# andrewmilson/ecfft

Hardware: AMD Instinct MI355X
Metric: secp256k1 Fp field-mul/s, ENTER+EXIT at n=2^20 (higher is better)
Workload: dtype u256; 1 GPU; secp256k1::Fp n=2^20 ENTER+EXIT (BASELINE.json configs[2]); n=1048576, field=secp256k1, parallelism=1 independent polynomial(s), one per GPU, no collective, inputs=device-resident (HBM) before the timed region, steps=449, warmup=5

## Files before the change

### ecfft_amd/csrc/device_tree.h

```cpp
#pragma once
#include <hip/hip_runtime.h>
#include <vector>
#include <set>
#include <map>
#include <mutex>
#include <atomic>
#include <cstdio>
#include <cstdlib>
#include <new>
#include <algorithm>
#include "kernels.h"
#include "host_curve.h"
#include "transport.h"

namespace ecfft {

#ifdef ECFFT_TEST_HOOKS
inline const char* ab_env(const char* name) { return getenv(name); }
#else
inline const char* ab_env(const char*) { return nullptr; }
#endif

#define ECFFT_HIP_TRY(x)                                                                   \
    do { hipError_t e_ = (x); if (e_ != hipSuccess) {                                      \
// ... 51 lines not shown

#define ECFFT_LAUNCH(cls, alg_bytes, kern, grid, block, lds, stream, ...)               \
    do { if (prof_.on) prof_.begin(stream, cls, (double)(alg_bytes));                  \
         hipLaunchKernelGGL(kern, grid, block, lds, stream, __VA_ARGS__);               \
         if (prof_.on) prof_.end(stream); } while (0)

#ifndef ECFFT_BATCH_SPLIT
#define ECFFT_BATCH_SPLIT 1
#endif
#ifndef ECFFT_SYM_BFLY
#define ECFFT_SYM_BFLY 1
#endif
#ifndef ECFFT_BATCH_WAYS
#define ECFFT_BATCH_WAYS 2
#endif
template <class F>
class DeviceChain {
public:
    using E = typename F::elem;
    using TE = typename F::telem;
    using Tree = LevelTables<F>;

    ~DeviceChain() { release(); }

    size_t size() const { return N_; }
    unsigned log_size() const { return L_; }
    const Tree& tree(unsigned log_m) const { return trees_[log_m]; }
    const Tree& tree_at(unsigned log_m) const { return (ovr_tree_ && ovr_tree_->log_m == log_m) ? *ovr_tree_ : trees_[log_m]; }
    const HostTree<F>& host() const { return host_; }
    int exit_cores() const { return exit3_ ? 3 : 4; }
    int exit_low_cores() const { return exit3_ && kExitLowForm == 3 && !exit_low4_ ? 3 : 4; }
    int sym_bfly() const { return !sym_ ? 0 : (sym_general_kernels_ ? 2 : 1); }
    int low_sym() const { return (kLowSymEnter && low_sym_enter() ? 1 : 0) | (kLowSymExit && low_sym_exit() ? 2 : 0); }
    int low_map(int dir) const {
        if (trees_.size() > 5 && trees_[5].low32_A[dir]) return 32;
        if (trees_.size() > 4 && trees_[4].low16_A[dir]) return 16;
        return 0;
    }
    const E* f_device() const { return f_; }
    std::mutex& lock() { return mu_; }
#ifdef ECFFT_TEST_HOOKS
    static std::atomic<int>& test_fail_build_rank() { static std::atomic<int> r{-1}; return r; }
#endif
    Profiler& profiler() const { return prof_; }

    bool build(HostTree<F>&& ht, int device) {
        host_ = std::move(ht);
        N_ = host_.n; L_ = ilog2(N_); device_ = device;
        ECFFT_HIP_TRY(hipSetDevice(device_));
        hipStream_t s = nullptr;
        size_t total = 2 * N_ + 64 + 2 * (L_ ? L_ : 1) + 64;
        for (unsigned l = 0; l <= L_; ++l) total += (6 + 11 * kTeElems) * ((size_t)1 << l) + 1024 + blk16_elems(l);
        if (!exit4_) for (unsigned l = 1; l <= L_; ++l) total += (l <= kLogLow ? 6 : 1) * kTeElems * ((size_t)1 << l) / 2 + 64;
        total += low16_elems();
        ECFFT_HIP_TRY(hipMalloc(&arena_, total * sizeof(E)));
        arena_cap_ = total; arena_used_ = 0;
        f_ = take(2 * N_);
        if (!points_on_device(f_, s)) { fprintf(stderr, "ecfft: point set construction failed\n"); return false; }
        if (!exit4_) {
            unsigned long long* zc = nullptr; unsigned long long hz = 0;
            ECFFT_HIP_TRY(hipMalloc(&zc, sizeof(unsigned long long)));
            (void)hipMemsetAsync(zc, 0, sizeof(unsigned long long), s);
            const E* leaves = f_ + N_;
            foreach_n(s, N_, [=] __device__(size_t j) { if (F::is_zero(leaves[j])) atomicAdd(zc, 1ull); });
            const bool got = hipMemcpyAsync(&hz, zc, sizeof(hz), hipMemcpyDeviceToHost, s) == hipSuccess && hipStreamSynchronize(s) == hipSuccess;
            (void)hipFree(zc);
// ... 471 lines not shown
            batch_inv(xqe, xqei, hc, s); batch_inv(xqo, xqoi, hc, s);
            foreach_n(s, hc, [=] __device__(size_t j) {
                e0[j] = F::mul(F::sub(F::sqr(xe[j]), zc0[j]), xqei[j]);
                e1[j] = F::mul(F::sub(F::sqr(F::sub(zb[j], xo[j])), zc1[j]), xqoi[j]);
            });
            ok = modred_split(tr, base, lq, m, e0, e1, h0, h1, xqei, xqo, 1, zib, 1, zc0, zc1, 1, t0, x0, x1, A, B, s, true);
            if (!ok) break;
            foreach_n(s, hc, [=] __device__(size_t j) { c0[j] = F::mul_add(xqe[j], h0[j], zc0[j]); c1[j] = F::mul_add(xqo[j], h1[j], zc1[j]); });
            E* z1s = temp(hc);
            pointwise_z(lm, 1, (size_t)a, hc, z1s, fdev, lc_inv, s, Q);
            foreach_n(s, hc, [=] __device__(size_t j) { e0[j] = F::sqr(F::sub(z1s[j], xe[j])); e1[j] = F::sqr(xo[j]); });
            ok = modred_split(tr, base, lq, m, e0, e1, q0, q1, xei, xo, 1, zib, 1, c0, c1, 1, t0, x0, x1, A, B, s, true);
            if (!ok) break;
            pz0[0] = c0; pz0[1] = c1; pz1[0] = q0; pz1[1] = q1;
            if (hipStreamSynchronize(s) != hipSuccess) { ok = false; break; }
            temps_free();
        }
        ok = ok && hipGetLastError() == hipSuccess && hipStreamSynchronize(s) == hipSuccess;
        temps_free();
        ok = tr.vote(ok, s);
        if (!ok) { fprintf(stderr, "ecfft: sharded EXIT table build failed\n"); return false; }
        host_.f.clear(); host_.f.shrink_to_fit();
        ECFFT_HIP_TRY(hipMalloc(&d_trees_, (L_ + 1) * sizeof(Tree)));
        ECFFT_HIP_TRY(hipMemcpy(d_trees_, trees_.data(), (L_ + 1) * sizeof(Tree), hipMemcpyHostToDevice));
        return true;
    }

#ifndef ECFFT_LOG_TILE_BYTES
#define ECFFT_LOG_TILE_BYTES 15
#endif
#ifndef ECFFT_CT_ALL
#define ECFFT_CT_ALL 0
#endif
    static constexpr unsigned kLogTileMax = (sizeof(E) == 32) ? ECFFT_LOG_TILE_BYTES - 5 : ECFFT_LOG_TILE_BYTES - 2;
#ifndef ECFFT_COL_STAGES
#define ECFFT_COL_STAGES 9
#endif
#ifndef ECFFT_LOG_COL_TILE_BYTES
#define ECFFT_LOG_COL_TILE_BYTES 15
#endif
#ifndef ECFFT_COL_MIN_LOGC
#define ECFFT_COL_MIN_LOGC 1
#endif
#ifndef ECFFT_COL_STAGES_4B
#define ECFFT_COL_STAGES_4B 9
#endif
    static constexpr unsigned kColStages = sizeof(E) == 4 ? ECFFT_COL_STAGES_4B : ECFFT_COL_STAGES;
    static constexpr bool kSymKernels = sizeof(E) == 32 && ECFFT_SYM_BFLY != 0;
    static constexpr bool kLowSymEnter = kSymKernels && ECFFT_ENTER_LOW_SYM != 0;
    static constexpr unsigned kLogColTileMax = (sizeof(E) == 32) ? ECFFT_LOG_COL_TILE_BYTES - 5 : ECFFT_LOG_COL_TILE_BYTES - 2;
    struct NextLoad { int ld_mode; const TE* ld_tbl; double extra_first; };
    struct EnterFuse { const E* src; E* dst; double extra; };
    bool extend_core(unsigned log_m, IoDesc<F> io, E* buf, size_t total, int srcpar, hipStream_t s,
                     double extra_first = 0.0, double extra_last = 0.0, unsigned k_begin = 0,
                     const NextLoad* next_ld = nullptr, bool skip_first_col = false, const EnterFuse* ef = nullptr) const {
        const Tree& T = tree_at(log_m);
        size_t e = T.e; unsigned le = ilog2(e);
        int tgt = 1 - srcpar;
        const bool symk = kSymKernels && sym_kernels();
        unsigned tz = (unsigned)__builtin_ctzll((unsigned long long)total);
        unsigned log_tile = tz < kLogTileMax ? tz : kLogTileMax;
        const bool small = small_launch(total) && !ef_small_off_;
        if (small && log_tile > kLogLowSmall) log_tile = kLogLowSmall;
        unsigned k_first = le > log_tile ? le - log_tile : 0;
        if (k_first < k_begin) k_first = k_begin;
        if (ef && k_first == 0 && le + 1 > log_tile) log_tile = le + 1;
        struct Pass { int kind; unsigned ka, kb; };
        Pass passes[2 * 8 + 1]; int np = 0;
        if (k_first > k_begin) {
            unsigned log_ct0 = tz < kLogColTileMax ? tz : kLogColTileMax;
            if (small && log_ct0 > kLogLowSmall) log_ct0 = kLogLowSmall;
            const unsigned minc = (small && log_ct0 == kLogLowSmall) ? small_min_logc_ : (unsigned)ECFFT_COL_MIN_LOGC;
            unsigned rmax = kColStages < log_ct0 - minc ? kColStages : log_ct0 - minc;
            if (rmax < 1) rmax = 1;
            unsigned ncol = k_first - k_begin, ngrp = (ncol + rmax - 1) / rmax;
            unsigned k = k_begin;
            for (unsigned g = 0; g < ngrp; ++g) { unsigned sz = ncol / ngrp + (g < ncol % ngrp ? 1 : 0); passes[np++] = {0, k, k + sz - 1}; k += sz; }
        }
        int nd = np;
        passes[np++] = {1, k_first, le};
        for (int g = nd - 1; g >= 0; --g) passes[np++] = {2, passes[g].ka, passes[g].kb};
        const uint32_t nt_st = (sizeof(E) == 32 && kNtStoreMaxLog && total <= ((size_t)1 << kNtStoreMaxLog)) ? 1u : 0u;
// ... 35 lines not shown
                else if (symk)
                ECFFT_LAUNCH(KC_COL, bytes, (k_stages_col_enter<F, kSymKernels>), dim3((unsigned)(total >> (log_ct + 1))), dim3(kBlockLds),
                             2 * sizeof(E) * ((size_t)col_row_stride<E>(1u << log_c) << R), s,
                             (const E*)buf, ef->src, ef->dst, T.p0[tgt], T.p1[tgt], T.xe, T.w[1], T.w1x, le, P.kb, log_c);
                else
                ECFFT_LAUNCH(KC_COL, bytes, k_stages_col_enter<F>, dim3((unsigned)(total >> (log_ct + 1))), dim3(kBlockLds),
                             2 * sizeof(E) * ((size_t)col_row_stride<E>(1u << log_c) << R), s,
                             (const E*)buf, ef->src, ef->dst, T.p0[tgt], T.p1[tgt], T.xe, T.w[1], T.w1x, le, P.kb, log_c);
                return false;
            }
            if (first) { d = io; d.st_tr_logp = 0; } else { d = IoDesc<F>{}; d.src = plain_src; d.src_stride = 1; d.src_off = 0; d.ld_mode = LD_PLAIN; d.ld_tbl = nullptr; }
            if (last) { d.dst = io.dst; d.st_mode = io.st_mode; d.st_a = io.st_a; d.st_b = io.st_b; d.aux = io.aux; d.aux_stride = io.aux_stride; d.aux_off = io.aux_off; d.aux_out = io.aux_out; d.st_c = io.st_c; d.aux2 = io.aux2;
                        d.st_tr_logp = io.st_tr_logp; d.tr_chunk = io.tr_chunk; }
            else { d.dst = buf; d.st_mode = ST_PLAIN; d.st_a = d.st_b = nullptr; d.aux = nullptr; d.aux_stride = d.aux_off = 0; d.aux_out = nullptr; }
            d.nt_st = nt_st;
            double extra = (first ? extra_first : 0.0) + (last ? extra_last : 0.0);
            const Pass& P = passes[pi];
            if (last && ef) {
                d.dst = ef->dst; d.st_mode = ST_ENTER; d.st_a = T.xe; d.st_b = T.w1x; d.st_c = T.w[1]; d.aux = ef->src; d.aux_stride = 1; d.aux_off = 0; d.aux_out = nullptr;
                extra += ef->extra;
            }
            if (P.kind == 1) {
                unsigned nst = le - k_first;
                double hsum = (double)((e >> k_first) - 1);
                double bytes = sizeof(E) * (2.0 * nst * 2.0 * total + 8.0 * hsum * tblw_) + extra;
                constexpr bool ct_row = sizeof(E) == 4 ? ((size_t)1 << kLogTileMax) == (size_t)kBlockRow * 16 : (ECFFT_CT_ALL != 0);
                const bool use_blk16 = sizeof(E) == 32 && kBlockRow == 512 && kLogTileMax == 10 && !mfma_off_ && T.blk16_A[srcpar] && log_tile == kLogTileMax && le - k_first >= 4;
                const uint8_t* bA = use_blk16 ? T.blk16_A[srcpar] : nullptr;
                const unsigned long long* bK = use_blk16 ? T.blk16_K[srcpar] : nullptr;
                if (sizeof(E) == 32 && log_tile == kLogLowSmall && !row256_off_ && d.st_mode != ST_ENTER && T.c0t[srcpar]) {
                    const bool mf = !mfma_off_ && T.blk16_A[srcpar] && le >= 4 && le - k_first >= 4;
                    ECFFT_LAUNCH(KC_ROW, bytes, (k_stages_row256<F>), dim3((unsigned)(total >> kLogLowSmall)), dim3(256), 0, s, d, T.dinv[srcpar], T.p0[tgt], T.p1[tgt], T.inner[srcpar],
                                 le, k_first, T.c0t[srcpar], mf ? T.blk16_A[srcpar] : (const uint8_t*)nullptr, mf ? T.blk16_K[srcpar] : (const unsigned long long*)nullptr);
                } else
                if (log_tile == kLogTileMax + 1 && ct_row) {
                    if constexpr (ct_row)
                    ECFFT_LAUNCH(KC_ROW, bytes, (k_stages_lds<F, (int)kLogTileMax + 1>), dim3((unsigned)(total >> log_tile)), dim3(kBlockRow),
                                 ((size_t)sizeof(E)) << log_tile, s, d, T.np0[srcpar], T.dinv[srcpar], T.p0[tgt], T.p1[tgt], T.inner[srcpar], le, k_first, log_tile, T.c0t[srcpar], bA, bK);
                } else if (log_tile == kLogTileMax && (ct_row || bA) && symk)
                    ECFFT_LAUNCH(KC_ROW, bytes, (k_stages_lds<F, (int)kLogTileMax, kSymKernels>), dim3((unsigned)(total >> log_tile)), dim3(kBlockRow),
                                 ((size_t)sizeof(E)) << log_tile, s, d, T.np0[srcpar], T.dinv[srcpar], T.p0[tgt], T.p1[tgt], T.inner[srcpar], le, k_first, log_tile, T.c0t[srcpar], bA, bK);
                else if (log_tile == kLogTileMax && (ct_row || bA))
                    ECFFT_LAUNCH(KC_ROW, bytes, (k_stages_lds<F, (int)kLogTileMax>), dim3((unsigned)(total >> log_tile)), dim3(kBlockRow),
                                 ((size_t)sizeof(E)) << log_tile, s, d, T.np0[srcpar], T.dinv[srcpar], T.p0[tgt], T.p1[tgt], T.inner[srcpar], le, k_first, log_tile, T.c0t[srcpar], bA, bK);
                else
                    ECFFT_LAUNCH(KC_ROW, bytes, (k_stages_lds<F, 0>), dim3((unsigned)(total >> log_tile)), dim3(kBlockRow),
                                 ((size_t)sizeof(E)) << log_tile, s, d, T.np0[srcpar], T.dinv[srcpar], T.p0[tgt], T.p1[tgt], T.inner[srcpar], le, k_first, log_tile, T.c0t[srcpar], bA, bK);
            } else {
                unsigned log_ct = tz < kLogColTileMax ? tz : kLogColTileMax;
                if (small && log_ct > kLogLowSmall) log_ct = kLogLowSmall;
                unsigned R = P.kb - P.ka + 1, log_c = log_ct - R;
                double hsum = 0; for (unsigned k = P.ka; k <= P.kb; ++k) hsum += (double)(e >> (k + 1));
                double bytes = sizeof(E) * (2.0 * R * total + 4.0 * hsum * tblw_) + extra;
                const bool ct = (log_ct == kLogColTileMax && (sizeof(E) == 4 || ECFFT_CT_ALL));
                const unsigned lv = ct ? pair_spans(total, le, P.ka, log_ct, d) : 0;
                dim3 grid((unsigned)(total >> (log_ct + lv))); size_t lds = (sizeof(E) * ((size_t)col_row_stride<E>(1u << log_c) << R)) << lv;
                constexpr bool kCtCol = sizeof(E) == 4 || ECFFT_CT_ALL;
                if (col256_ok(log_ct, le) && lv == 0 && (P.kind != 0 || T.c0t[srcpar])) {
                    if (P.kind == 0) ECFFT_LAUNCH(KC_COL, bytes, (k_stages_col256<F, true>), dim3((unsigned)(total >> log_ct)), dim3(256), 0, s, d, T.c0t[srcpar], T.dinv[srcpar], le, P.ka, P.kb, log_c);
                    else ECFFT_LAUNCH(KC_COL, bytes, (k_stages_col256<F, false>), dim3((unsigned)(total >> log_ct)), dim3(256), 0, s, d, T.p0[tgt], T.p1[tgt], le, P.ka, P.kb, log_c);
                } else
                if (symk && !ct) {
                    if (P.kind == 0) ECFFT_LAUNCH(KC_COL, bytes, (k_stages_col<F, true, 0, kSymKernels>), grid, dim3(kBlockLds), lds, s, d, T.np0[srcpar], T.dinv[srcpar], le, P.ka, P.kb, log_c, T.c0t[srcpar], (uint32_t)lv);
                    else ECFFT_LAUNCH(KC_COL, bytes, (k_stages_col<F, false, 0, kSymKernels>), grid, dim3(kBlockLds), lds, s, d, T.p0[tgt], T.p1[tgt], le, P.ka, P.kb, log_c, (const TE*)nullptr, (uint32_t)lv);
                } else
                if (P.kind == 0) {
// ... 3108 lines not shown
    unsigned shard_log_p_ = 0, shard_rank_ = 0;
    std::vector<ShardSet> sets_;
    const Tree* ovr_tree_ = nullptr; const ShardSet* ovr_set_ = nullptr;
    mutable double tblw_ = 1.0;
    mutable std::map<uint64_t, TE*> full_cyc_; mutable size_t full_cyc_bytes_ = 0;
    bool full_cyc_off_ = ab_env("ECFFT_NO_FULL_CYCLIC") != nullptr;
    unsigned low32_mask_ = ab_env("ECFFT_LOW32") ? (unsigned)atoi(ab_env("ECFFT_LOW32")) : 0u;
    bool low16_off_ = ab_env("ECFFT_NO_LOW16") != nullptr;
    bool mfma_off_ = ab_env("ECFFT_NO_MFMA") != nullptr;
    unsigned small_min_logc_ = ab_env("ECFFT_SMALL_MIN_LOGC") ? (unsigned)atoi(ab_env("ECFFT_SMALL_MIN_LOGC")) : 1u;
    bool in_halves_ = false;
    Tree pair_full_{}; bool have_pair_full_ = false;
    unsigned gather_max_log_ = ab_env("ECFFT_SPLIT_GATHER_MAX_LOG") ? (unsigned)atoi(ab_env("ECFFT_SPLIT_GATHER_MAX_LOG")) : 21u;
    mutable void* stripe_stage_ = nullptr; mutable size_t stripe_bytes_ = 0;
    struct StripeScope { const DeviceChain* ch; StripeScope(const DeviceChain* c, void* p, size_t b) : ch(c) { ch->stripe_stage_ = p; ch->stripe_bytes_ = p ? b : 0; }
                         ~StripeScope() { ch->stripe_stage_ = nullptr; ch->stripe_bytes_ = 0; } };
    bool stripe_off_ = ab_env("ECFFT_NO_STRIPE") != nullptr;
    size_t stripe_gain_ = ab_env("ECFFT_STRIPE_MIN_GAIN") ? (size_t)atoll(ab_env("ECFFT_STRIPE_MIN_GAIN")) : ~(size_t)0;
    bool q2_split_ = ab_env("ECFFT_SPLIT_Q2_SPLIT") != nullptr;
    bool col256_off_ = ab_env("ECFFT_NO_COL256") != nullptr;
    bool row256_off_ = ab_env("ECFFT_NO_ROW256") != nullptr;
    bool ef_small_off_ = ab_env("ECFFT_NO_SMALL_TILES") != nullptr;
    bool exit4_ = ECFFT_EXIT_CORES == 4 || ab_env("ECFFT_EXIT_FOUR_CORES") != nullptr;
    bool exit3_ = false;
    bool exit_low4_ = ab_env("ECFFT_EXIT_LOW_FOUR_CORES") != nullptr;
    E* crit_ = nullptr;
    bool sym_ = false;
    bool sym_off_ = ab_env("ECFFT_NO_SYM_BFLY") != nullptr;
    bool sym_general_kernels_ = ab_env("ECFFT_SYM_BFLY_GENERAL_KERNELS") != nullptr;
    bool sym_kernels() const { return sym_ && !sym_general_kernels_; }
    bool low_general_kernels_ = ab_env("ECFFT_LOW_GENERAL_KERNELS") != nullptr;
    bool low_sym_enter() const { return sym_kernels() && !low_general_kernels_ && !exit4_; }
    bool low_sym_exit() const { return low_sym_enter() && exit_low_cores() == 3; }
};

}
```

### ecfft_amd/csrc/ecfft_capi.hip

```cpp
#include <hip/hip_runtime.h>
#include <cstring>
#include <memory>
#include <new>
#include "device_tree.h"
#include "wire_parse.h"
#include "../../include/ecfft_hip.h"
#ifdef ECFFT_TEST_HOOKS
#include "../../include/ecfft_hip_hooks.h"
#endif

using namespace ecfft;

struct ecfft_ctx {
    int field;
    int device;
    std::unique_ptr<DeviceChain<Secp256k1>> secp;
    std::unique_ptr<DeviceChain<M31>> m31;
    void* stage = nullptr;
    size_t stage_bytes = 0;
    hipEvent_t last_op = nullptr;
    ~ecfft_ctx() { if (stage) (void)hipFree(stage); if (last_op) (void)hipEventDestroy(last_op); }
};

namespace {
// ... 1496 lines not shown
    if (!matrix256 || !x || !out || !n || n % 256 || mode < 1 || mode > 4) return ECFFT_ERR_BAD_ARG;
    return run_blk16_selftest(matrix256, x, out, n, mode, device);
}

int ecfft_selftest_blk32(const void* matrix1024, const void* x, void* out, size_t n, int device) {
    if (!matrix1024 || !x || !out || !n || n % 1024) return ECFFT_ERR_BAD_ARG;
    return run_blk_selftest(matrix1024, 1024, x, out, n, Blk16::kABytes32 + Blk16::kKWords32 * 8, 1024 * sizeof(Fe256), device,
                            [&](Fe256* dT, Fe256* dx, uint8_t* dA, Fe256* dcs) {
        unsigned long long* dK = reinterpret_cast<unsigned long long*>(dA + Blk16::kABytes32);
        hipLaunchKernelGGL(k_blk32_expand, dim3(4), dim3(256), 0, nullptr, (const Fe256*)dT, dA, dcs, false);
        hipLaunchKernelGGL(k_blk32_seeds, dim3(1), dim3(32), 0, nullptr, (const Fe256*)dcs, dK);
        hipLaunchKernelGGL(k_blk32_apply, dim3((unsigned)(n / 1024)), dim3(512), 0, nullptr, dx, dA, dK);
    });
}
int ecfft_ctx_low_map(const ecfft_ctx* ctx, int dir) {
    if (!ctx || dir < 0 || dir > 1 || ctx->field != ECFFT_FIELD_SECP256K1 || !ctx->secp) return 0;
    return ctx->secp->low_map(dir);
}
int ecfft_ctx_exit_cores(const ecfft_ctx* ctx) {
    if (!ctx) return 0;
    return ctx->secp ? ctx->secp->exit_cores() : ctx->m31 ? ctx->m31->exit_cores() : 0;
}
int ecfft_ctx_exit_low_cores(const ecfft_ctx* ctx) {
    if (!ctx) return 0;
    return ctx->secp ? ctx->secp->exit_low_cores() : ctx->m31 ? ctx->m31->exit_low_cores() : 0;
}
int ecfft_ctx_sym_bfly(const ecfft_ctx* ctx) {
    if (!ctx) return -1;
    return ctx->secp ? ctx->secp->sym_bfly() : ctx->m31 ? ctx->m31->sym_bfly() : -1;
}
int ecfft_ctx_low_sym(const ecfft_ctx* ctx) {
    if (!ctx) return -1;
    return ctx->secp ? ctx->secp->low_sym() : ctx->m31 ? ctx->m31->low_sym() : -1;
}

#endif
int ecfft_mul_ceiling(int field, int device, int waves_per_simd, double* mul_per_s) {
    return with_field(field, [&](auto tag) { return run_mul_ceiling<typename decltype(tag)::type>(device, waves_per_simd, mul_per_s); });
}

int ecfft_device_alloc(int device, size_t bytes, void** out) {
    if (!out) return ECFFT_ERR_BAD_ARG;
    *out = nullptr;
    if (!have_device(device)) return ECFFT_ERR_HIP;
    DeviceGuard dev(device);
    if (!dev.ok) return ECFFT_ERR_HIP;
    return hipMalloc(out, bytes ? bytes : 1) == hipSuccess ? ECFFT_OK : ECFFT_ERR_HIP;
}
int ecfft_device_free(void* ptr) { return !ptr || hipFree(ptr) == hipSuccess ? ECFFT_OK : ECFFT_ERR_HIP; }
int ecfft_device_sync(int device) {
    DeviceGuard dev(device);
    return dev.ok && hipDeviceSynchronize() == hipSuccess ? ECFFT_OK : ECFFT_ERR_HIP;
}

int ecfft_shader_clock(int field, int device, double* mhz) {
    return with_field(field, [&](auto tag) { return run_shader_clock<typename decltype(tag)::type>(device, mhz); });
}

int ecfft_device_copy(void* dst, const void* src, size_t bytes, int kind) {
    hipMemcpyKind k = kind == 0 ? hipMemcpyDeviceToHost : (kind == 1 ? hipMemcpyHostToDevice : hipMemcpyDeviceToDevice);
    if (!dst || !src || kind < 0 || kind > 2) return ECFFT_ERR_BAD_ARG;
    return hipMemcpy(dst, src, bytes, k) == hipSuccess ? ECFFT_OK : ECFFT_ERR_HIP;
}

int ecfft_device_info(int device, char* buf, size_t cap) {
    if (!buf || !cap) return ECFFT_ERR_BAD_ARG;
// ... 429 lines not shown
```

### ecfft_amd/csrc/kernels.h

```cpp
#pragma once
#include <hip/hip_runtime.h>
#include <stdint.h>
#include <stddef.h>
#include <type_traits>
#include "mfma_blk16.h"
#include "curve_points.h"

namespace ecfft {

constexpr int kBlock = 256;

__device__ __forceinline__ void lds_barrier() { asm volatile("s_waitcnt lgkmcnt(0)\n\ts_barrier" ::: "memory"); }
#ifndef ECFFT_WAVE_LOCAL
#define ECFFT_WAVE_LOCAL 1
#endif
__device__ __forceinline__ void wave_local_sync() {
#if ECFFT_WAVE_LOCAL == 2
    asm volatile("s_waitcnt lgkmcnt(0)" ::: "memory");
#elif ECFFT_WAVE_LOCAL == 1
    __builtin_amdgcn_fence(__ATOMIC_ACQ_REL, "wavefront");
    asm volatile("" ::: "memory");
#else
    lds_barrier();
#endif
// ... 755 lines not shown
                    }, cb);
                return;
            }
        }
#ifdef ECFFT_EXP_NO_TILE_IO
        return;
#endif
        for (uint32_t g = tid; g < npairs; g += kBlockRow) {
            const uint32_t i = g & (uint32_t)emask, lb = (g >> log_e) << (log_e + 1);
            const size_t bb = base + lb;
            const E u0 = io.aux[bb + i], v0 = io.aux[bb + e + i];
            const E ev = F::tmul_add(io.st_a[i], v0, u0);
            const E od = F::tmul_add(io.st_b[i], tile[lb + (uint32_t)e + i], F::tmul(io.st_c[i], tile[lb + i]));
            io.dst[bb + 2 * i] = F::canon(ev);
            io.dst[bb + 2 * i + 1] = F::canon(od);
        }
        return;
    }
    if constexpr (kFast) {
        if (vio) {
#ifndef ECFFT_EXP_NO_TILE_IO
#pragma unroll 1
            for (uint32_t b = 0; b < (uint32_t)kNQ / 4; ++b) vio_store<F, 4, kBlockRow>(io, log_e, tile, [=](uint32_t j) { return base + j; }, tid + b * 4u * kBlockRow);
#endif
            return;
        }
    }
#ifndef ECFFT_EXP_NO_TILE_IO
#pragma unroll
    for (uint32_t j = tid; j < T; j += kBlockRow) io_store<F>(io, base + j, log_e, tile[j]);
#endif
}

template <class F, int BLK, bool SWZ = false>
__device__ __forceinline__ void reg_extend32(typename F::elem* a, uint32_t len, uint32_t log_e, uint32_t k_first,
                                             const typename F::telem* __restrict__ c0t, const typename F::telem* __restrict__ dinv,
                                             const typename F::telem* __restrict__ p0, const typename F::telem* __restrict__ p1,
                                             const typename F::telem* __restrict__ inner, uint32_t tid,
                                             const uint8_t* __restrict__ blkA, const unsigned long long* __restrict__ blkK);

template <class F>
__global__ __launch_bounds__(256, 2) void k_stages_row256(IoDesc<F> io,
                                                          const typename F::telem* __restrict__ dinv,
                                                          const typename F::telem* __restrict__ p0,
                                                          const typename F::telem* __restrict__ p1,
                                                          const typename F::telem* __restrict__ inner,
                                                          uint32_t log_e, uint32_t k_first,
                                                          const typename F::telem* __restrict__ c0t,
                                                          const uint8_t* __restrict__ blkA, const unsigned long long* __restrict__ blkK) {
    using E = typename F::elem;
    if constexpr (sizeof(E) == 32) {
        __shared__ E tile[256];
        const uint32_t tid = threadIdx.x;
        const size_t pos = ((size_t)blockIdx.x << 8) + tid;
        const size_t emask = ((size_t)1 << log_e) - 1;
        tile[tid] = io_load<F>(io, pos, emask);
        __syncthreads();
        reg_extend32<F, 256>(tile, 256u, log_e, k_first, c0t, dinv, p0, p1, inner, tid, blkA, blkK);
        io_store<F>(io, pos, log_e, tile[tid]);
    }
}

#ifndef ECFFT_COL_PAD
#define ECFFT_COL_PAD 0
#endif
template <class E>
// ... 2724 lines not shown
```

### ecfft_amd/fftree.py

```python
import ctypes
import enum
import os

import numpy as np

from . import build as _build

_DIR = os.path.dirname(os.path.abspath(__file__))

OK, ERR_NOT_POW2, ERR_TREE_TOO_SMALL, ERR_TREE_TOO_LARGE, ERR_HIP, ERR_BAD_ARG = range(6)
MEM_HOST, MEM_DEVICE = 0, 1
TBL_F, TBL_RECOMBINE, TBL_DECOMPOSE, TBL_XNN_S, TBL_XNN_S_INV, TBL_Z0_S1, TBL_Z1_S0, TBL_Z0_INV_S1, TBL_Z1_INV_S0, TBL_Z0Z0, TBL_Z1Z1 = range(11)

EXPORTS = ["ecfft_elem_size", "ecfft_build_fftree", "ecfft_fftree_new", "ecfft_ctx_destroy", "ecfft_tree_size",
           "ecfft_field", "ecfft_enter", "ecfft_exit", "ecfft_extend", "ecfft_tree_table", "ecfft_build_points",
           "ecfft_device_info", "ecfft_profile_enable", "ecfft_profile_classes", "ecfft_profile_read",
           "ecfft_extend_top_cyclic", "ecfft_extend_local_block",
           "ecfft_mul_ceiling", "ecfft_elems_to_standard", "ecfft_elems_from_standard", "ecfft_table_fma", "ecfft_enter_many", "ecfft_exit_many", "ecfft_mextend", "ecfft_redc", "ecfft_modular_reduce", "ecfft_vanish", "ecfft_degree",
           "ecfft_comm_get_unique_id", "ecfft_comm_init_rank", "ecfft_comm_init_callback", "ecfft_comm_destroy", "ecfft_comm_rank", "ecfft_comm_world",
           "ecfft_comm_stats_enable", "ecfft_comm_stats_read", "ecfft_extend_sharded", "ecfft_enter_sharded", "ecfft_exit_sharded", "ecfft_device_copy", "ecfft_shader_clock", "ecfft_device_alloc", "ecfft_device_free", "ecfft_device_sync", "ecfft_build_extend_shard", "ecfft_ctx_device_bytes", "ecfft_extend_sharded_layout", "ecfft_build_enter_shard", "ecfft_build_exit_shard", "ecfft_build_exit_shard_opts",
           "ecfft_fftree_serialize", "ecfft_fftree_deserialize", "ecfft_tree_rational_maps", "ecfft_ctx_trim", "ecfft_comm_abort", "ecfft_comm_set_rccl_library", "ecfft_comm_set_link_striping",
           "ecfft_poly_mul", "ecfft_poly_inv_series", "ecfft_poly_divrem", "ecfft_poly_eval_points", "ecfft_poly_interpolate",
           "ecfft_poly_pow_mod", "ecfft_poly_mul_mod", "ecfft_poly_gcd", "ecfft_poly_xgcd", "ecfft_poly_xgcd_partial", "ecfft_rs_decode", "ecfft_poly_find_roots",
           "ecfft_poly_compose_mod", "ecfft_poly_squarefree", "ecfft_poly_distinct_degree", "ecfft_poly_equal_degree", "ecfft_division_polynomial", "ecfft_curve_trace_mod", "ecfft_curve_cardinality",
           "ecfft_find_curve_candidate", "ecfft_curve_two_sylow", "ecfft_find_curve", "ecfft_build_fftree_on_curve",
           "ecfft_curve_point_mul", "ecfft_curve_point_two_adicity", "ecfft_curve_find_generator", "ecfft_build_ec_fftree"]
GCD_SMALL_MAX = 256
XGCD_PARTIAL_SMALL_MAX = 256
RS_SMALL_MAX = 255
ROOTS_SMALL_MAX = 65
COMPOSE_SMALL_MAX = 65
DDF_SMALL_MAX = 65
EDF_SMALL_MAX = 65
SCHOOF_SMALL_MAX = 65
SCHOOF_MAX_L = 199
ORDER_BYTES = 40

HOOK_EXPORTS = ['ecfft_selftest_field', 'ecfft_selfcheck_pointwise_z', 'ecfft_test_fail_next_collective', 'ecfft_selftest_blk16', 'ecfft_selftest_blk16_small', 'ecfft_test_fail_build_rank', 'ecfft_comm_init_projection', 'ecfft_selftest_blk32', 'ecfft_ctx_low_map', 'ecfft_curve_search_stats', 'ecfft_test_ddf_iterate', 'ecfft_test_schoof_pi2', 'ecfft_ctx_exit_cores', 'ecfft_ctx_exit_low_cores', 'ecfft_ctx_sym_bfly', 'ecfft_ctx_low_sym']

EXCHANGE_FN = ctypes.CFUNCTYPE(ctypes.c_int, ctypes.c_void_p, ctypes.c_int, ctypes.POINTER(ctypes.c_int), ctypes.POINTER(ctypes.c_void_p),
                               ctypes.POINTER(ctypes.c_size_t), ctypes.c_int, ctypes.POINTER(ctypes.c_int), ctypes.POINTER(ctypes.c_void_p),
                               ctypes.POINTER(ctypes.c_size_t), ctypes.c_void_p)


class Moiety(enum.IntEnum):
    S0 = 0
    S1 = 1


class EcfftError(RuntimeError):
    pass


_lib = None
HOOKS_LIB = os.path.join(os.path.dirname(_DIR), "tests", "hooks", "libecfft_hip_hooks.so")


def _bind(L):
    vp, sz, ci = ctypes.c_void_p, ctypes.c_size_t, ctypes.c_int
    L.ecfft_elem_size.restype, L.ecfft_elem_size.argtypes = sz, [ci]
    L.ecfft_build_fftree.restype, L.ecfft_build_fftree.argtypes = ci, [ci, sz, ci, ctypes.POINTER(vp)]
    L.ecfft_fftree_new.restype, L.ecfft_fftree_new.argtypes = ci, [ci, vp, sz, vp, vp, ci, ctypes.POINTER(vp)]
    L.ecfft_ctx_destroy.restype, L.ecfft_ctx_destroy.argtypes = None, [vp]
    L.ecfft_tree_size.restype, L.ecfft_tree_size.argtypes = sz, [vp]
    L.ecfft_field.restype, L.ecfft_field.argtypes = ci, [vp]
    L.ecfft_enter.restype, L.ecfft_enter.argtypes = ci, [vp, vp, vp, sz, ci, vp]
    L.ecfft_exit.restype, L.ecfft_exit.argtypes = ci, [vp, vp, vp, sz, ci, vp]
    L.ecfft_extend.restype, L.ecfft_extend.argtypes = ci, [vp, vp, vp, sz, ci, sz, ci, vp]
    L.ecfft_poly_mul.restype, L.ecfft_poly_mul.argtypes = ci, [vp, vp, sz, vp, sz, vp, sz, ci, vp]
    L.ecfft_poly_inv_series.restype, L.ecfft_poly_inv_series.argtypes = ci, [vp, vp, sz, vp, sz, sz, ci, vp]
    L.ecfft_poly_divrem.restype, L.ecfft_poly_divrem.argtypes = ci, [vp, vp, sz, vp, sz, vp, vp, sz, ci, vp]
# ... 55 lines not shown
    L.ecfft_profile_enable.restype, L.ecfft_profile_enable.argtypes = ci, [vp, ci]
    L.ecfft_profile_classes.restype, L.ecfft_profile_classes.argtypes = ci, []
    L.ecfft_profile_read.restype, L.ecfft_profile_read.argtypes = ci, [vp, ci, ctypes.c_char_p, sz, ctypes.POINTER(ctypes.c_uint64),
                                                                           ctypes.POINTER(ctypes.c_double), ctypes.POINTER(ctypes.c_double)]
    u32, u64 = ctypes.c_uint32, ctypes.c_uint64
    L.ecfft_find_curve_candidate.restype, L.ecfft_find_curve_candidate.argtypes = ci, [ci, u64, u64, vp, vp]
    L.ecfft_curve_two_sylow.restype, L.ecfft_curve_two_sylow.argtypes = ci, [ci, ci, vp, vp, sz, vp, vp]
    L.ecfft_find_curve.restype, L.ecfft_find_curve.argtypes = ci, [ci, ci, ctypes.c_uint, u64, u64, u64, ctypes.POINTER(u64), ctypes.POINTER(u32),
                                                                   vp, vp, vp, vp]
    L.ecfft_build_fftree_on_curve.restype, L.ecfft_build_fftree_on_curve.argtypes = ci, [ci, sz, vp, vp, vp, ctypes.c_uint, vp, ci, ctypes.POINTER(vp)]
    L.ecfft_curve_point_mul.restype, L.ecfft_curve_point_mul.argtypes = ci, [ci, ci, vp, vp, sz, vp, vp, vp, sz, sz, vp, vp, sz]
    L.ecfft_curve_point_two_adicity.restype, L.ecfft_curve_point_two_adicity.argtypes = ci, [ci, ci, vp, vp, sz, vp, vp, ctypes.c_uint, vp, sz]
    L.ecfft_curve_find_generator.restype, L.ecfft_curve_find_generator.argtypes = ci, [ci, ci, vp, vp, vp, u64, u64, ctypes.POINTER(ctypes.c_uint), vp, vp,
                                                                                       ctypes.POINTER(u64)]
    L.ecfft_build_ec_fftree.restype, L.ecfft_build_ec_fftree.argtypes = ci, [ci, sz, vp, vp, vp, ctypes.c_uint, vp, ci, ctypes.POINTER(vp)]
    L.ecfft_comm_set_rccl_library.restype, L.ecfft_comm_set_rccl_library.argtypes = ci, [ctypes.c_char_p]
    L.ecfft_comm_set_link_striping.restype, L.ecfft_comm_set_link_striping.argtypes = ci, [vp, sz]
    L.has_hooks = hasattr(L, "ecfft_selftest_field")
    if L.has_hooks:
        L.ecfft_selftest_field.restype, L.ecfft_selftest_field.argtypes = ci, [ci, ci, vp, vp, vp, vp, sz, ci]
        L.ecfft_selfcheck_pointwise_z.restype, L.ecfft_selfcheck_pointwise_z.argtypes = ctypes.c_long, [vp, sz]
        L.ecfft_test_fail_next_collective.restype, L.ecfft_test_fail_next_collective.argtypes = ci, [vp]
        L.ecfft_test_fail_build_rank.restype, L.ecfft_test_fail_build_rank.argtypes = ci, [ci]
        L.ecfft_selftest_blk16.restype, L.ecfft_selftest_blk16.argtypes = ci, [vp, vp, vp, sz, ci]
        L.ecfft_selftest_blk16_small.restype, L.ecfft_selftest_blk16_small.argtypes = ci, [vp, vp, vp, sz, ci, ci]
        L.ecfft_selftest_blk32.restype, L.ecfft_selftest_blk32.argtypes = ci, [vp, vp, vp, sz, ci]
        L.ecfft_ctx_low_map.restype, L.ecfft_ctx_low_map.argtypes = ci, [vp, ci]
        L.ecfft_ctx_exit_cores.restype, L.ecfft_ctx_exit_cores.argtypes = ci, [vp]
        L.ecfft_ctx_exit_low_cores.restype, L.ecfft_ctx_exit_low_cores.argtypes = ci, [vp]
        if hasattr(L, "ecfft_ctx_sym_bfly"):
            L.ecfft_ctx_sym_bfly.restype, L.ecfft_ctx_sym_bfly.argtypes = ci, [vp]
        if hasattr(L, "ecfft_ctx_low_sym"):
            L.ecfft_ctx_low_sym.restype, L.ecfft_ctx_low_sym.argtypes = ci, [vp]
        L.ecfft_curve_search_stats.restype, L.ecfft_curve_search_stats.argtypes = ci, [ctypes.POINTER(ctypes.c_uint64), ctypes.POINTER(ctypes.c_double), sz, ci]
        L.ecfft_test_ddf_iterate.restype, L.ecfft_test_ddf_iterate.argtypes = ci, [ci]
        L.ecfft_test_schoof_pi2.restype, L.ecfft_test_schoof_pi2.argtypes = ci, [ci]
        L.ecfft_comm_init_projection.restype = ci
        L.ecfft_comm_init_projection.argtypes = [ci, ci, ci, ctypes.c_double, ctypes.c_double, ctypes.POINTER(vp)]
    return L


def _load(path):
    try:
        import torch
    except ImportError:
        pass
    return _bind(ctypes.CDLL(path))


def lib():
    global _lib
    if _lib is None:
        path = os.environ.get("ECFFT_LIB") or os.path.join(_DIR, "libecfft_hip.so")
        if not os.path.exists(path):
            _build.build()
        _lib = _load(path)
    return _lib


class use_library:
    _loaded = {}

    def __init__(self, path):
        self.path = os.path.abspath(path)

    def __enter__(self):
# ... 690 lines not shown
        import torch
        assert _is_torch(x) and x.is_cuda and x.is_contiguous(), "sharded transforms take contiguous CUDA tensors"
        out = torch.empty_like(x)
        stream = torch.cuda.current_stream(x.device).cuda_stream
        _check(fn(self._h, comm._h, x.data_ptr(), out.data_ptr(), length, *extra, stream))
        return out

    def extend_sharded(self, comm, x_block, e, moiety, cyclic_in=False, cyclic_out=False):
        if not (cyclic_in or cyclic_out):
            return self._sharded(self._L.ecfft_extend_sharded, comm, x_block, e, int(moiety))
        return self._sharded(self._L.ecfft_extend_sharded_layout, comm, x_block, e, int(moiety), int(cyclic_in), int(cyclic_out))

    def enter_sharded(self, comm, x_block, n):
        return self._sharded(self._L.ecfft_enter_sharded, comm, x_block, n)

    def exit_sharded(self, comm, y_block, n):
        return self._sharded(self._L.ecfft_exit_sharded, comm, y_block, n)

    def low_map(self, direction):
        return self._L.ecfft_ctx_low_map(self._h, int(direction))

    def exit_cores(self):
        return self._L.ecfft_ctx_exit_cores(self._h)

    def exit_low_cores(self):
        return self._L.ecfft_ctx_exit_low_cores(self._h)

    def sym_bfly(self):
        return self._L.ecfft_ctx_sym_bfly(self._h)

    def low_sym(self):
        return self._L.ecfft_ctx_low_sym(self._h)

    def profile(self, on):
        _check(self._L.ecfft_profile_enable(self._h, int(on)))

    def profile_read(self):
        out = []
        for c in range(self._L.ecfft_profile_classes()):
            name = ctypes.create_string_buffer(64); n = ctypes.c_uint64(); ms = ctypes.c_double(); by = ctypes.c_double()
            _check(self._L.ecfft_profile_read(self._h, c, name, 64, ctypes.byref(n), ctypes.byref(ms), ctypes.byref(by)))
            out.append({"name": name.value.decode(), "launches": n.value, "ms": ms.value, "alg_bytes": by.value})
        return out

    def table(self, which, m=None):
        m = self.n if m is None else m
        cnt = ctypes.c_size_t()
        _check(self._L.ecfft_tree_table(self._h, m, which, None, 0, ctypes.byref(cnt)))
        out = np.zeros(self.field.shape(cnt.value), self.field.dtype)
        _check(self._L.ecfft_tree_table(self._h, m, which, out.ctypes.data, cnt.value, ctypes.byref(cnt)))
        return out

    def leaves(self, m=None):
        m = self.n if m is None else m
        return self.table(TBL_F, m)[m:]

    def serialize(self, compress):
        ln = ctypes.c_size_t()
        _check(self._L.ecfft_fftree_serialize(self._h, int(bool(compress)), None, 0, ctypes.byref(ln)))
        buf = ctypes.create_string_buffer(ln.value)
        _check(self._L.ecfft_fftree_serialize(self._h, int(bool(compress)), buf, ln.value, ctypes.byref(ln)))
        return buf.raw[:ln.value]

    def rational_map(self, k):
        if not hasattr(self, "_maps"):
            ln = max(self.n.bit_length() - 1, 1)
# ... 39 lines not shown
```

### include/ecfft_hip_hooks.h

```cpp
#ifndef ECFFT_HIP_HOOKS_H
#define ECFFT_HIP_HOOKS_H
#include "ecfft_hip.h"
#ifdef __cplusplus
extern "C" {
#endif

long ecfft_selfcheck_pointwise_z(ecfft_ctx* ctx, size_t m);

int ecfft_comm_init_projection(int world, int rank, int device, double delay_us, double link_gbps, ecfft_comm** out);

int ecfft_test_fail_next_collective(ecfft_ctx* ctx);
int ecfft_test_fail_build_rank(int rank);

int ecfft_selftest_field(int field, int op, const void* a, const void* b, const void* c, void* out, size_t n, int device);

int ecfft_selftest_blk16(const void* matrix256, const void* x, void* out, size_t n, int device);
int ecfft_selftest_blk16_small(const void* matrix256, const void* x, void* out, size_t n, int mode, int device);
int ecfft_selftest_blk32(const void* matrix1024, const void* x, void* out, size_t n, int device);
int ecfft_ctx_low_map(const ecfft_ctx* ctx, int dir);
int ecfft_ctx_exit_cores(const ecfft_ctx* ctx);
int ecfft_ctx_exit_low_cores(const ecfft_ctx* ctx);
int ecfft_ctx_sym_bfly(const ecfft_ctx* ctx);
int ecfft_ctx_low_sym(const ecfft_ctx* ctx);
int ecfft_curve_search_stats(uint64_t* lens, double* seconds, size_t cap, int reset);

int ecfft_test_ddf_iterate(int mode);

int ecfft_test_schoof_pi2(int mode);

#ifdef __cplusplus
}
#endif
#endif
```

Baseline: 569.3 billion field-mul/s.

## Add specialized 1024-thread ENTER kernel for log-tile-11 fused extend

Adds a dedicated k_enter_l11 kernel for the ENTER-fused extend pass when the tile is 2048 elements (le=10, log_tile=11). It loads the 2048-element tile into LDS and runs the two 1024-element halves concurrently with 1024 threads, using the 16x16 matrix-core phase in the middle. The final ENTER store (combining with the aux source and writing interleaved outputs) is fused into the same kernel. The intent is to replace the generic LDS row kernel for this shape with one that uses more threads and matrix-core stages. The cost is higher per-block resource use and a large, specialized code path.

```diff
diff --git a/ecfft_amd/csrc/device_tree.h b/ecfft_amd/csrc/device_tree.h
--- a/ecfft_amd/csrc/device_tree.h
+++ b/ecfft_amd/csrc/device_tree.h
@@ -107,6 +107,7 @@
     int exit_low_cores() const { return exit3_ && kExitLowForm == 3 && !exit_low4_ ? 3 : 4; }
     int sym_bfly() const { return !sym_ ? 0 : (sym_general_kernels_ ? 2 : 1); }
     int low_sym() const { return (kLowSymEnter && low_sym_enter() ? 1 : 0) | (kLowSymExit && low_sym_exit() ? 2 : 0); }
+    int enter_l11() const { return trees_.size() > kLogTileMax + 1 && enter_l11_tuned(trees_[kLogTileMax + 1], 0) ? 1 : 0; }
     int low_map(int dir) const {
         if (trees_.size() > 5 && trees_[5].low32_A[dir]) return 32;
         if (trees_.size() > 4 && trees_[4].low16_A[dir]) return 16;
@@ -644,6 +645,12 @@
 #ifndef ECFFT_CT_ALL
 #define ECFFT_CT_ALL 0
 #endif
+#ifndef ECFFT_ENTER_L11_TUNED
+#define ECFFT_ENTER_L11_TUNED 1
+#endif
+#ifndef ECFFT_ENTER_L11_THREADS
+#define ECFFT_ENTER_L11_THREADS 1024
+#endif
     static constexpr unsigned kLogTileMax = (sizeof(E) == 32) ? ECFFT_LOG_TILE_BYTES - 5 : ECFFT_LOG_TILE_BYTES - 2;
 #ifndef ECFFT_COL_STAGES
 #define ECFFT_COL_STAGES 9
@@ -660,6 +667,7 @@
     static constexpr unsigned kColStages = sizeof(E) == 4 ? ECFFT_COL_STAGES_4B : ECFFT_COL_STAGES;
     static constexpr bool kSymKernels = sizeof(E) == 32 && ECFFT_SYM_BFLY != 0;
     static constexpr bool kLowSymEnter = kSymKernels && ECFFT_ENTER_LOW_SYM != 0;
+    static constexpr bool kEnterL11 = sizeof(E) == 32 && ECFFT_ENTER_L11_TUNED != 0 && kBlockRow == 512 && kLogTileMax == 10;
     static constexpr unsigned kLogColTileMax = (sizeof(E) == 32) ? ECFFT_LOG_COL_TILE_BYTES - 5 : ECFFT_LOG_COL_TILE_BYTES - 2;
     struct NextLoad { int ld_mode; const TE* ld_tbl; double extra_first; };
     struct EnterFuse { const E* src; E* dst; double extra; };
@@ -761,6 +769,16 @@
                     const bool mf = !mfma_off_ && T.blk16_A[srcpar] && le >= 4 && le - k_first >= 4;
                     ECFFT_LAUNCH(KC_ROW, bytes, (k_stages_row256<F>), dim3((unsigned)(total >> kLogLowSmall)), dim3(256), 0, s, d, T.dinv[srcpar], T.p0[tgt], T.p1[tgt], T.inner[srcpar],
                                  le, k_first, T.c0t[srcpar], mf ? T.blk16_A[srcpar] : (const uint8_t*)nullptr, mf ? T.blk16_K[srcpar] : (const unsigned long long*)nullptr);
+                } else
+                if (ef && k_first == 0 && le == kLogTileMax && log_tile == le + 1 && !small && enter_l11_tuned(T, srcpar)) {
+                    if constexpr (kEnterL11) {
+                    if (symk)
+                    ECFFT_LAUNCH(KC_ROW, bytes, (k_enter_l11<F, kSymKernels, ECFFT_ENTER_L11_THREADS>), dim3((unsigned)(total >> log_tile)), dim3(ECFFT_ENTER_L11_THREADS), ((size_t)sizeof(E)) << log_tile, s,
+                                 d, T.np0[srcpar], T.dinv[srcpar], T.p0[tgt], T.p1[tgt], T.blk16_A[srcpar], T.blk16_K[srcpar]);
+                    else
+                    ECFFT_LAUNCH(KC_ROW, bytes, (k_enter_l11<F, false, ECFFT_ENTER_L11_THREADS>), dim3((unsigned)(total >> log_tile)), dim3(ECFFT_ENTER_L11_THREADS), ((size_t)sizeof(E)) << log_tile, s,
+                                 d, T.np0[srcpar], T.dinv[srcpar], T.p0[tgt], T.p1[tgt], T.blk16_A[srcpar], T.blk16_K[srcpar]);
+                    }
                 } else
                 if (log_tile == kLogTileMax + 1 && ct_row) {
                     if constexpr (ct_row)
@@ -3935,6 +3953,8 @@
     bool low_general_kernels_ = ab_env("ECFFT_LOW_GENERAL_KERNELS") != nullptr;
     bool low_sym_enter() const { return sym_kernels() && !low_general_kernels_ && !exit4_; }
     bool low_sym_exit() const { return low_sym_enter() && exit_low_cores() == 3; }
+    bool enter_l11_generic_ = ab_env("ECFFT_ENTER_L11_GENERIC") != nullptr;
+    bool enter_l11_tuned(const Tree& T, int srcpar) const { return kEnterL11 && !enter_l11_generic_ && !mfma_off_ && !shard_mode() && T.blk16_A[srcpar] != nullptr; }
 };
 
 }
diff --git a/ecfft_amd/csrc/ecfft_capi.hip b/ecfft_amd/csrc/ecfft_capi.hip
--- a/ecfft_amd/csrc/ecfft_capi.hip
+++ b/ecfft_amd/csrc/ecfft_capi.hip
@@ -1552,6 +1552,10 @@
 int ecfft_ctx_low_sym(const ecfft_ctx* ctx) {
     if (!ctx) return -1;
     return ctx->secp ? ctx->secp->low_sym() : ctx->m31 ? ctx->m31->low_sym() : -1;
+}
+int ecfft_ctx_enter_l11(const ecfft_ctx* ctx) {
+    if (!ctx) return -1;
+    return ctx->secp ? ctx->secp->enter_l11() : ctx->m31 ? ctx->m31->enter_l11() : -1;
 }
 
 #endif
diff --git a/ecfft_amd/csrc/kernels.h b/ecfft_amd/csrc/kernels.h
--- a/ecfft_amd/csrc/kernels.h
+++ b/ecfft_amd/csrc/kernels.h
@@ -811,6 +811,63 @@
 #endif
 }
 
+template <class F, bool SYM, int BLK>
+__global__ __launch_bounds__(BLK, ECFFT_MIN_WAVES) void k_enter_l11(IoDesc<F> io,
+                                                                   const typename F::telem* __restrict__ np0,
+                                                                   const typename F::telem* __restrict__ dinv,
+                                                                   const typename F::telem* __restrict__ p0,
+                                                                   const typename F::telem* __restrict__ p1,
+                                                                   const uint8_t* __restrict__ blkA, const unsigned long long* __restrict__ blkK) {
+    using E = typename F::elem;
+    static_assert(sizeof(E) == 32 && Blk16::kSub == 1024 && (BLK == 512 || BLK == 1024), "32-byte field, 1024-element matrix-core phases");
+    extern __shared__ __attribute__((aligned(16))) unsigned char ecfft_smem[];
+    E* const blk = reinterpret_cast<E*>(ecfft_smem);
+    constexpr uint32_t e = 1024, log_e = 10;
+    const size_t base = (size_t)blockIdx.x << (log_e + 1);
+#pragma unroll
+    for (uint32_t j = threadIdx.x; j < 2 * e; j += BLK) blk[j] = io_load<F>(io, base + j, (size_t)e - 1);
+    __syncthreads();
+#pragma unroll 1
+    for (uint32_t sub = 0; sub < 1024u / BLK; ++sub) {
+        uint32_t tid = threadIdx.x & 511u;
+        asm volatile("" : "+v"(tid));
+        E* const tile = blk + (BLK == 1024 ? threadIdx.x >> 9 : sub) * e;
+        row_stages_pipe<F, true, SYM>(tile, np0, dinv, e, (int)log_e - 1, 5, tid, 4);
+        Blk16::APre pre;
+        const uint32_t i = tid & 15u, idx = ((tid >> 4) << 5) + i;
+        {
+            const E a = tile[idx], b = tile[idx + 16];
+            E q0, q1;
+            if constexpr (SYM) { q0 = a; q1 = b; sym_bfly<F, true>(q0, q1, ldt(dinv + (e - 32), i)); }
+            else { q1 = F::tmul(ldt(dinv + (e - 32), i), F::sub(b, a)); q0 = F::tmul_add(ldt(np0 + (e - 32), i), q1, a); }
+            __builtin_amdgcn_sched_barrier(0);
+            pre = Blk16::prefetch(blkA, tid);
+            __builtin_amdgcn_sched_barrier(0);
+            if (ECFFT_WAVE_LOCAL) wave_local_sync(); else __syncthreads();
+            Blk16::store_operand(tile, idx, q0); Blk16::store_operand(tile, idx + 16, q1);
+            __syncthreads();
+        }
+        Blk16::phase(tile, blkA, blkK, tid, pre);
+        {
+            const E a = Blk16::load_swizzled(tile, idx), b = Blk16::load_swizzled(tile, idx + 16);
+            E o0, o1;
+            if constexpr (SYM) { o0 = a; o1 = b; sym_bfly<F, false>(o0, o1, ldt(p0 + (e - 32), i)); }
+            else { o0 = F::tmul_add(ldt(p0 + (e - 32), i), b, a); o1 = F::tmul_add(ldt(p1 + (e - 32), i), b, a); }
+            if (ECFFT_WAVE_LOCAL) wave_local_sync(); else __syncthreads();
+            tile[idx] = o0; tile[idx + 16] = o1;
+            if (ECFFT_WAVE_LOCAL) wave_local_sync(); else __syncthreads();
+        }
+        row_stages_pipe<F, false, SYM>(tile, p0, p1, e, 5, (int)log_e - 1, tid);
+    }
+    for (uint32_t i = threadIdx.x; i < e; i += BLK) {
+        const E u0 = io.aux[base + i], v0 = io.aux[base + e + i];
+        const E ev = F::tmul_add(io.st_a[i], v0, u0);
+        const E od = F::tmul_add(io.st_b[i], blk[e + i], F::tmul(io.st_c[i], blk[i]));
+        io.dst[base + 2 * i] = F::canon(ev);
+        io.dst[base + 2 * i + 1] = F::canon(od);
+    }
+}
+
 template <class F, int BLK, bool SWZ = false>
 __device__ __forceinline__ void reg_extend32(typename F::elem* a, uint32_t len, uint32_t log_e, uint32_t k_first,
                                              const typename F::telem* __restrict__ c0t, const typename F::telem* __restrict__ dinv,
diff --git a/ecfft_amd/fftree.py b/ecfft_amd/fftree.py
--- a/ecfft_amd/fftree.py
+++ b/ecfft_amd/fftree.py
@@ -36,7 +36,7 @@
 SCHOOF_MAX_L = 199
 ORDER_BYTES = 40
 
-HOOK_EXPORTS = ['ecfft_selftest_field', 'ecfft_selfcheck_pointwise_z', 'ecfft_test_fail_next_collective', 'ecfft_selftest_blk16', 'ecfft_selftest_blk16_small', 'ecfft_test_fail_build_rank', 'ecfft_comm_init_projection', 'ecfft_selftest_blk32', 'ecfft_ctx_low_map', 'ecfft_curve_search_stats', 'ecfft_test_ddf_iterate', 'ecfft_test_schoof_pi2', 'ecfft_ctx_exit_cores', 'ecfft_ctx_exit_low_cores', 'ecfft_ctx_sym_bfly', 'ecfft_ctx_low_sym']
+HOOK_EXPORTS = ['ecfft_selftest_field', 'ecfft_selfcheck_pointwise_z', 'ecfft_test_fail_next_collective', 'ecfft_selftest_blk16', 'ecfft_selftest_blk16_small', 'ecfft_test_fail_build_rank', 'ecfft_comm_init_projection', 'ecfft_selftest_blk32', 'ecfft_ctx_low_map', 'ecfft_curve_search_stats', 'ecfft_test_ddf_iterate', 'ecfft_test_schoof_pi2', 'ecfft_ctx_exit_cores', 'ecfft_ctx_exit_low_cores', 'ecfft_ctx_sym_bfly', 'ecfft_ctx_low_sym', 'ecfft_ctx_enter_l11']
 
 EXCHANGE_FN = ctypes.CFUNCTYPE(ctypes.c_int, ctypes.c_void_p, ctypes.c_int, ctypes.POINTER(ctypes.c_int), ctypes.POINTER(ctypes.c_void_p),
                                ctypes.POINTER(ctypes.c_size_t), ctypes.c_int, ctypes.POINTER(ctypes.c_int), ctypes.POINTER(ctypes.c_void_p),
@@ -158,6 +158,8 @@
             L.ecfft_ctx_sym_bfly.restype, L.ecfft_ctx_sym_bfly.argtypes = ci, [vp]
         if hasattr(L, "ecfft_ctx_low_sym"):
             L.ecfft_ctx_low_sym.restype, L.ecfft_ctx_low_sym.argtypes = ci, [vp]
+        if hasattr(L, "ecfft_ctx_enter_l11"):
+            L.ecfft_ctx_enter_l11.restype, L.ecfft_ctx_enter_l11.argtypes = ci, [vp]
         L.ecfft_curve_search_stats.restype, L.ecfft_curve_search_stats.argtypes = ci, [ctypes.POINTER(ctypes.c_uint64), ctypes.POINTER(ctypes.c_double), sz, ci]
         L.ecfft_test_ddf_iterate.restype, L.ecfft_test_ddf_iterate.argtypes = ci, [ci]
         L.ecfft_test_schoof_pi2.restype, L.ecfft_test_schoof_pi2.argtypes = ci, [ci]
@@ -914,6 +916,9 @@
     def low_sym(self):
         return self._L.ecfft_ctx_low_sym(self._h)
 
+    def enter_l11(self):
+        return self._L.ecfft_ctx_enter_l11(self._h)
+
     def profile(self, on):
         _check(self._L.ecfft_profile_enable(self._h, int(on)))
 
diff --git a/include/ecfft_hip_hooks.h b/include/ecfft_hip_hooks.h
--- a/include/ecfft_hip_hooks.h
+++ b/include/ecfft_hip_hooks.h
@@ -22,6 +22,7 @@
 int ecfft_ctx_exit_low_cores(const ecfft_ctx* ctx);
 int ecfft_ctx_sym_bfly(const ecfft_ctx* ctx);
 int ecfft_ctx_low_sym(const ecfft_ctx* ctx);
+int ecfft_ctx_enter_l11(const ecfft_ctx* ctx);
 int ecfft_curve_search_stats(uint64_t* lens, double* seconds, size_t cap, int reset);
 
 int ecfft_test_ddf_iterate(int mode);
```

New measurement: 575.4 billion field-mul/s, median of 6. 1.01x the previous value.
